# Patman86/SVT-AV1-Mod-by-Patman

Measured on AMD Instinct MI355X. Metric: encoded fps (4K 10-bit preset 8) + ME+txfm HBM GB/s vs roofline, 1/2/4/8 GPU, higher is better.
Workload: dtype u8 (ME) / int32 (transform)

## Files before the change

svt-av1-mod-by-patman_amd/csrc/me_frame.hip:

```cpp
#include <cstdio>
#include <cstdlib>
#include <cstring>

#include "common.hpp"
#include "sad_device.hpp"

using namespace svthip;
using namespace svthip::dev;

namespace {

#define NL 2
#define NR 4
#define MAX_SAD_VALUE_ (128 * 128 * 255)
#define MAX_U32_ 0xFFFFFFFFu

constexpr uint32_t ME_HME_WIN_DW = 3200;
constexpr uint32_t ME_WIN_DW     = ME_HME_WIN_DW - 64 * 16 - 256;
constexpr uint32_t fp_pitch_c(uint32_t tw) { return (((tw + 3) >> 2) + 17) | 1u; }
constexpr uint32_t FP_TILE_W = ME_WIN_DW / fp_pitch_c(64) >= 63 + 8 ? 64 : 32;
static_assert(ME_WIN_DW / fp_pitch_c(FP_TILE_W) >= 63 + 8, "full-pel window buffer too small for one tile");

struct PreHme {
    uint64_t sad;
    uint16_t sa_w, sa_h;
    int16_t  col, row;
    uint8_t  valid, pad_[7];
};

struct B64State {
    uint32_t org_x, org_y, b64_w, b64_h;
    SvtHipMeSearchResult sr[NL][NR];
    uint32_t reduce_div[NL][NR];
    uint32_t zz_sad[NL][NR];
    PreHme   ph[NL][NR][2];
    uint8_t  performed_phme[NL][NR][2];
    int16_t  l0x[NL][NR][2][2], l0y[NL][NR][2][2], l1x[NL][NR][2][2], l1y[NL][NR][2][2], l2x[NL][NR][2][2],
        l2y[NL][NR][2][2];
    uint64_t l0s[NL][NR][2][2], l1s[NL][NR][2][2], l2s[NL][NR][2][2];
    SvtHipSearchArea l0_min, l0_max;
    uint32_t wg_sum;
    int16_t  xc, yc, sw, sh, ox, oy;
    int32_t  do_centre, need_zero_sad, need_hme_sad;
    int16_t  stx, sty, stw, sth;
    int32_t  staged, restage;
    uint32_t zero_sad, hme_mv_sad;
    int16_t  fp_xc[NL * NR], fp_yc[NL * NR], fp_sw[NL * NR], fp_sh[NL * NR], fp_ox[NL * NR], fp_oy[NL * NR];
    uint8_t  fp_centre[NL * NR];
    uint32_t fp_inv[NL * NR];
    uint32_t first_ref_sad64;
    uint64_t me_sad_sum[NL][NR];
};

struct MeLds {
    static constexpr uint32_t WIN_DW = ME_WIN_DW, HME_WIN_DW = ME_HME_WIN_DW;
    SearchShared sh;
    B64State     st;
    union {
        alignas(16) uint32_t win[ME_HME_WIN_DW];
        struct {
            alignas(16) uint32_t fp_win_[ME_WIN_DW];
            alignas(16) uint32_t src_full[64 * 16];
            uint64_t bestkey[85];
            uint32_t me_dist[85];
        };
    };
    alignas(16) uint32_t src_q[32 * 8];
    alignas(16) uint32_t src_s[16 * 4];
};
static_assert(sizeof(MeLds::win) >= (ME_WIN_DW + 64 * 16) * 4 + 85 * 12, "full-pel view must fit the HME window buffer");

typedef __attribute__((address_space(1))) uint32_t g_u32;
#define MINV(a, b) ((a) < (b) ? (a) : (b))
#define MAXV(a, b) ((a) > (b) ? (a) : (b))
#define ABSV(a) ((a) < 0 ? -(a) : (a))

__device__ __forceinline__ uint32_t div_small(uint32_t x, uint32_t d) {
    return (d & (d - 1u)) == 0u && d ? x >> (31u - (uint32_t)__builtin_clz(d)) : x / d;
}

__device__ __forceinline__ uint16_t scaled_dist(uint16_t dist) {
    return (uint16_t)(((dist * 5) / 8) + ((dist % 8) == 0 ? 0 : 1));
}
__device__ __forceinline__ uint16_t pic_dist(const SvtHipMeParams &p, int li, int ri) {
    const int64_t d = (int64_t)p.picture_number - (int64_t)p.ref_picture_number[li][ri];
    return (uint16_t)(int16_t)ABSV(d);
}
__device__ __forceinline__ const uint8_t *plane_at(const SvtHipPlane8 &pl, int x, int y) {
    return pl.buf + (ptrdiff_t)((int)pl.org_y + y) * (ptrdiff_t)pl.stride + (int)pl.org_x + x;
}

__device__ __forceinline__ uint32_t block_sad16(const uint32_t *src, const uint8_t *ref, uint32_t ref_stride, uint32_t ndw, uint32_t rows,
                                                uint32_t row_step, uint32_t lane, uint32_t nlanes) {
    const uint32_t nch = (ndw + 3) >> 2, inv = make_inv_small(nch);
    uint32_t       acc = 0;
    for (uint32_t idx = lane; idx < nch * rows; idx += nlanes) {
        const uint32_t r = fast_div(idx, inv), ch = idx - r * nch;
        const uint4    sv = *(const uint4 *)&src[(r * row_step) * 16 + 4 * ch];
        const u128v    v  = load_u128_any(ref + (size_t)sad_mul_u24(r * row_step, ref_stride) + 16 * ch);
        const uint32_t nd = ndw - 4 * ch;
        acc = __builtin_amdgcn_sad_u8(sv.x, v.x, acc);
        acc = __builtin_amdgcn_sad_u8(sv.y, v.y, acc);
        if (nd > 2) {
            acc = __builtin_amdgcn_sad_u8(sv.z, v.z, acc);
            acc = __builtin_amdgcn_sad_u8(sv.w, v.w, acc);
        }
    }
    return acc;
}

template <class LDS>
__device__ void wg_block_sad(LDS &L, const uint8_t *ref, uint32_t ref_stride, uint32_t width, uint32_t rows,
                             uint32_t row_step) {
    if (threadIdx.x == 0)
        L.st.wg_sum = 0;
    __syncthreads();
    uint32_t acc = block_sad16(L.src_full, ref, ref_stride, width >> 2, rows, row_step, threadIdx.x, blockDim.x);
    acc = wave_sum(acc);
    if ((threadIdx.x & 63) == 0)
        atomicAdd(&L.st.wg_sum, acc);
    __syncthreads();
}

__device__ void hme_clamp(int16_t org_x, int16_t org_y, int16_t pad_w, int16_t pad_h, int16_t W, int16_t H, int16_t *pox,
                          int16_t *poy, int16_t *pw, int16_t *ph) {
    int16_t ox = *pox, oy = *poy, sa_w = *pw, sa_h = *ph;
    if ((org_x + ox) < -pad_w) {
        ox   = (int16_t)(-pad_w - org_x);
        sa_w = (int16_t)(sa_w - (-pad_w - (org_x + ox)));
    }
    if ((org_x + ox) > W - 1)
        ox = (int16_t)(ox - ((org_x + ox) - (W - 1)));
    if ((org_x + ox + sa_w) > W)
        sa_w = (int16_t)MAXV(1, sa_w - ((org_x + ox + sa_w) - W));
    sa_w = (sa_w < 8) ? sa_w : (int16_t)(sa_w & ~0x07);
    if ((org_y + oy) < -pad_h) {
        oy   = (int16_t)(-pad_h - org_y);
        sa_h = (int16_t)(sa_h - (-pad_h - (org_y + oy)));
    }
    if ((org_y + oy) > H - 1)
        oy = (int16_t)(oy - ((org_y + oy) - (H - 1)));
    if ((org_y + oy + sa_h) > H)
        sa_h = (int16_t)MAXV(1, sa_h - ((org_y + oy + sa_h) - H));
    *pox = ox, *poy = oy, *pw = sa_w, *ph = sa_h;
}

__device__ void set_desc(SearchDesc &d, const SvtHipMeParams &p, const SvtHipPlane8 &rp, int x_tl, int y_tl, int16_t sa_w,
                         int16_t sa_h, uint32_t skip) {
    const bool full = p.hme_search_method == 1;
    d.ref           = rp.buf + (ptrdiff_t)y_tl * (ptrdiff_t)rp.stride + x_tl;
    d.ref_stride    = full ? rp.stride : rp.stride * 2;
    d.raw_stride    = rp.stride;
    d.sa_w          = sa_w;
    d.sa_h          = sa_h;
    d.skip          = skip;
}

template <class SH>
__device__ void decode_result(const SH &sh, uint32_t i, bool sub, uint64_t *sad, int16_t *x, int16_t *y) {
    const uint64_t key = sh.best[i];
    uint64_t       s   = key >> 32;
    if (key != KEY_NONE) {
        const uint32_t idx = (uint32_t)key;
        *x = (int16_t)(idx & 0xffffu);
        *y = (int16_t)(idx >> 16);
    }
    if (sub)
        s *= 2;
    *sad = s;
}

__device__ void set_quadrants(int16_t x[2][2], int16_t y[2][2], uint64_t s[2][2], int16_t vx, int16_t vy, uint64_t vs) {
    for (int a = 0; a < 2; a++)
        for (int b = 0; b < 2; b++) x[a][b] = vx, y[a][b] = vy, s[a][b] = vs;
}

__device__ void best_quadrant(int16_t x[2][2], int16_t y[2][2], uint64_t s[2][2], int16_t *bx, int16_t *by, uint64_t *bs) {
    *bx = x[0][0], *by = y[0][0], *bs = s[0][0];
    if (s[1][0] < *bs) *bx = x[1][0], *by = y[1][0], *bs = s[1][0];
    if (s[0][1] < *bs) *bx = x[0][1], *by = y[0][1], *bs = s[0][1];
    if (s[1][1] < *bs) *bx = x[1][1], *by = y[1][1], *bs = s[1][1];
}

__device__ void clamp_me_window(int16_t xc, int16_t yc, int16_t ox_b, int16_t oy_b, int16_t W, int16_t H, int16_t pad, int16_t *psw,
                                int16_t *psh, int16_t *pox, int16_t *poy) {
    int16_t sw = *psw, sh_ = *psh;
    int16_t ox = (int16_t)(xc - (sw >> 1)), oy = (int16_t)(yc - (sh_ >> 1));
    ox  = ((ox_b + ox) < -pad) ? (int16_t)(-pad - ox_b) : ox;
    sw  = ((ox_b + ox) < -pad) ? (int16_t)(sw - (-pad - (ox_b + ox))) : sw;
    ox  = ((ox_b + ox) > W - 1) ? (int16_t)(ox - ((ox_b + ox) - (W - 1))) : ox;
    sw  = ((ox_b + ox + sw) > W) ? (int16_t)MAXV(1, sw - ((ox_b + ox + sw) - W)) : sw;
    sw  = (sw < 8) ? sw : (int16_t)(sw & ~0x07);
    oy  = ((oy_b + oy) < -pad) ? (int16_t)(-pad - oy_b) : oy;
    sh_ = ((oy_b + oy) < -pad) ? (int16_t)(sh_ - (-pad - (oy_b + oy))) : sh_;
    oy  = ((oy_b + oy) > H - 1) ? (int16_t)(oy - ((oy_b + oy) - (H - 1))) : oy;
    sh_ = ((oy_b + oy + sh_) > H) ? (int16_t)MAXV(1, sh_ - ((oy_b + oy + sh_) - H)) : sh_;
    *psw = sw, *psh = sh_, *pox = ox, *poy = oy;
}

__device__ __forceinline__ uint32_t fp_pitch(uint32_t tw) { return (((tw + 3) >> 2) + 17) | 1u; }

template <class LDS>
__device__ void fp_stage(LDS &L, const uint8_t *win_org, uint32_t stride, uint32_t tw, uint32_t th) {
    stage_rows16(L.win, fp_pitch(tw), win_org, stride, th + 63, blockDim.x, threadIdx.x);
    __syncthreads();
}

template <int CTRL> __device__ __forceinline__ uint32_t dpp_add(uint32_t v) {
    return v + (uint32_t)__builtin_amdgcn_update_dpp(0, (int)v, CTRL, 0xf, 0xf, false);
}

template <class LDS>
__device__ void fp_search(LDS &L, uint32_t pitch, uint32_t x0, uint32_t y0, uint32_t cw, uint32_t ch, uint32_t order0,
                          uint32_t order_pitch, bool sub) {
    const uint32_t tid = threadIdx.x;
    const uint32_t nq = (cw + 3) >> 2, nitems = nq * ch * 16, inv_nq = make_inv_small(nq);
    const uint32_t zo = tid & 15;
    const uint32_t zy = 2 * (zo >> 3) + ((zo >> 1) & 1), zx = 2 * ((zo >> 2) & 1) + (zo & 1);
    const uint32_t *s = &L.src_full[(16 * zy) * 16 + 4 * zx];
    for (uint32_t base = 0; base < nitems; base += blockDim.x) {
        if (base + (tid & ~63u) >= nitems)
            break;
        const uint32_t item = base + tid;
        const bool     on   = item < nitems;
        const uint32_t qi = on ? item >> 4 : 0, y = fast_div(qi, inv_nq), q = qi - sad_mul_u24(y, nq);
        const uint32_t *w = &L.win[sad_mul_u24(y0 + y + 16 * zy, pitch) + (x0 >> 2) + q + 4 * zx];
        uint64_t        a00 = 0, a01 = 0, a10 = 0, a11 = 0;
#pragma unroll
        for (uint32_t r = 0; r < 16; r++) {
            if (sub && (r & 1))
                continue;
            const uint32_t d0 = w[r * pitch], d1 = w[r * pitch + 1], d2 = w[r * pitch + 2], d3 = w[r * pitch + 3], d4 = w[r * pitch + 4];
            const uint4    sv = *(const uint4 *)&s[r * 16];
            if (r < 8) {
                a00 = __builtin_amdgcn_qsad_pk_u16_u8(pair64(d0, d1), sv.x, a00);
                a00 = __builtin_amdgcn_qsad_pk_u16_u8(pair64(d1, d2), sv.y, a00);
                a01 = __builtin_amdgcn_qsad_pk_u16_u8(pair64(d2, d3), sv.z, a01);
                a01 = __builtin_amdgcn_qsad_pk_u16_u8(pair64(d3, d4), sv.w, a01);
            } else {
                a10 = __builtin_amdgcn_qsad_pk_u16_u8(pair64(d0, d1), sv.x, a10);
                a10 = __builtin_amdgcn_qsad_pk_u16_u8(pair64(d1, d2), sv.y, a10);
                a11 = __builtin_amdgcn_qsad_pk_u16_u8(pair64(d2, d3), sv.z, a11);
                a11 = __builtin_amdgcn_qsad_pk_u16_u8(pair64(d3, d4), sv.w, a11);
            }
        }
        uint32_t k8[4] = {~0u, ~0u, ~0u, ~0u}, k16 = ~0u, k32 = ~0u, k64 = ~0u;
#pragma unroll
        for (uint32_t pp = 0; pp < 4; pp++) {
            const uint32_t lo_hi_shift = 16 * (pp & 1);
            const uint32_t c0 = ((pp < 2 ? (uint32_t)a00 : (uint32_t)(a00 >> 32)) >> lo_hi_shift) & 0xffff;
            const uint32_t c1 = ((pp < 2 ? (uint32_t)a01 : (uint32_t)(a01 >> 32)) >> lo_hi_shift) & 0xffff;
            const uint32_t c2 = ((pp < 2 ? (uint32_t)a10 : (uint32_t)(a10 >> 32)) >> lo_hi_shift) & 0xffff;
            const uint32_t c3 = ((pp < 2 ? (uint32_t)a11 : (uint32_t)(a11 >> 32)) >> lo_hi_shift) & 0xffff;
            const uint32_t s16 = c0 + c1 + c2 + c3;
            uint32_t       s32 = dpp_add<0xB1>(s16);
            s32                = dpp_add<0x4E>(s32);
            uint32_t s64       = dpp_add<0x124>(s32);
            s64                = dpp_add<0x128>(s64);
            if (4 * q + pp < cw) {
                k8[0] = min(k8[0], (c0 << 2) | pp), k8[1] = min(k8[1], (c1 << 2) | pp);
                k8[2] = min(k8[2], (c2 << 2) | pp), k8[3] = min(k8[3], (c3 << 2) | pp);
                k16 = min(k16, (s16 << 2) | pp), k32 = min(k32, (s32 << 2) | pp), k64 = min(k64, (s64 << 2) | pp);
            }
        }
        if (on && k16 != ~0u) {
            const uint32_t sh1 = sub ? 1 : 0;
            const uint32_t ord_row = order0 + sad_mul_u24(y, order_pitch) + 4 * q;
#define FP_KEY(k) (((unsigned long long)(((k) >> 2) << sh1) << 32) | (ord_row + ((k) & 3u)))
#pragma unroll
            for (uint32_t c = 0; c < 4; c++) atomicMin((unsigned long long *)&L.bestkey[21 + 4 * zo + c], FP_KEY(k8[c]));
            atomicMin((unsigned long long *)&L.bestkey[5 + zo], FP_KEY(k16));
            if ((zo & 3) == 0)
                atomicMin((unsigned long long *)&L.bestkey[1 + (zo >> 2)], FP_KEY(k32));
            if (zo == 0)
                atomicMin((unsigned long long *)&L.bestkey[0], FP_KEY(k64));
#undef FP_KEY
        }
    }
    __syncthreads();
}

__device__ const uint8_t z_to_raster_d[85] = {
    0,  1,  2,  3,  4,  5,  6,  9,  10, 7,  8,  11, 12, 13, 14, 17, 18, 15, 16, 19, 20, 21, 22, 29, 30, 23, 24, 31, 32,
    37, 38, 45, 46, 39, 40, 47, 48, 25, 26, 33, 34, 27, 28, 35, 36, 41, 42, 49, 50, 43, 44, 51, 52, 53, 54, 61, 62, 55,
    56, 63, 64, 69, 70, 77, 78, 71, 72, 79, 80, 57, 58, 65, 66, 59, 60, 67, 68, 73, 74, 81, 82, 75, 76, 83, 84};
__device__ __forceinline__ uint8_t pack_cand(uint32_t direction, uint32_t l0, uint32_t l1, uint32_t r0, uint32_t r1) {
    return (uint8_t)((direction & 3) | ((l0 & 3) << 2) | ((l1 & 3) << 4) | ((r0 & 1) << 6) | ((r1 & 1) << 7));
}
__device__ __forceinline__ int use_me_pu(const SvtHipMeParams &p, uint32_t n) {
    return p.enable_me_16x16 ? (p.enable_me_8x8 || n < 21) : (n < 5);
}

#define GS(li, ri, n) gs[((li) * NR + (ri)) * 85 + (n)]
#define GM(li, ri, n) gm[((li) * NR + (ri)) * 85 + (n)]

template <class LDS>
// ... 820 lines not shown
        fp_stage(L, plane_at(rp, ox_b + S.stx, oy_b + S.sty), rp.stride, (uint32_t)S.stw, (uint32_t)S.sth);
        fp_search(L, fp_pitch((uint32_t)S.stw), (uint32_t)(S.xc - S.stx), (uint32_t)(S.yc - S.sty), 1, 1, 0, 1, me_sub);
        if (tid < 64) {
            const uint32_t v    = (uint32_t)(L.bestkey[21 + tid] >> 32);
            const uint32_t mean = (uint32_t)(L.bestkey[0] >> 32) / 64;
            const int32_t  dv   = (int32_t)v - (int32_t)mean;
            const uint32_t ssq  = wave_sum((uint32_t)(dv * dv));
            if (tid == 0) {
                int16_t        sw = S.sw, sh_ = S.sh;
                const uint32_t var = ssq / 64;
                if (var > p.me_sr_mult2_th) {
                    sw  = (int16_t)((MAXV(1, sw * 3 / 2) + 7) & ~0x7);
                    sh_ = (int16_t)MAXV(1, sh_ * 3 / 2);
                }
                if (var < p.me_sr_div4_th) {
                    sw  = (int16_t)((MAXV(1, sw >> 2) + 7) & ~0x7);
                    sh_ = (int16_t)MAXV(1, sh_ >> 2);
                    sh_ = (int16_t)MAXV(3, sh_);
                } else if (var < p.me_sr_div2_th) {
                    sw  = (int16_t)((MINV(sw, sw >> 1) + 7) & ~0x7);
                    sh_ = (int16_t)MINV(sh_, sh_ >> 1);
                    sh_ = (int16_t)MAXV(3, sh_);
                }
                S.sw = sw, S.sh = sh_;
            }
        }
        __syncthreads();
    }
    if (tid == 0) {
        int16_t sw = S.sw, sh_ = S.sh, ox, oy;
        clamp_me_window(S.xc, S.yc, ox_b, oy_b, W, H, pad, &sw, &sh_, &ox, &oy);
        S.sw = sw, S.sh = sh_, S.ox = ox, S.oy = oy;
        S.restage = !(S.staged && ox >= S.stx && oy >= S.sty && ox + (sw > 0 ? sw : 0) <= S.stx + S.stw &&
                      oy + (sh_ > 0 ? sh_ : 0) <= S.sty + S.sth && ((ox - S.stx) & 3) == 0);
    }
    __syncthreads();
    }
    {
        const int      ox = S.ox, oy = S.oy;
        const uint32_t sw = (uint32_t)(S.sw > 0 ? S.sw : 0), sh_ = (uint32_t)(S.sh > 0 ? S.sh : 0);
        if (!S.restage) {
            fp_search(L, fp_pitch((uint32_t)S.stw), (uint32_t)(ox - S.stx), (uint32_t)(oy - S.sty), sw, sh_, 1, sw, me_sub);
        } else {
            const uint32_t tw = sw < FP_TILE_W ? sw : FP_TILE_W;
            const uint32_t pitch_t = fp_pitch(tw);
            uint32_t       th      = tw ? MINV(sh_, LDS::WIN_DW / pitch_t - 63) : 0;
            for (uint32_t ty = 0; th && ty < sh_; ty += th)
                for (uint32_t tx = 0; tx < sw; tx += tw) {
                    const uint32_t cw = MINV(tw, sw - tx), ch = MINV(th, sh_ - ty);
                    fp_stage(L, plane_at(rp, ox_b + ox + (int)tx, oy_b + oy + (int)ty), rp.stride, cw, ch);
                    fp_search(L, fp_pitch(cw), 0, 0, cw, ch, 1 + ty * sw + tx, sw, me_sub);
                }
        }
        uint32_t part = 0;
        for (uint32_t pu = tid; pu < 85; pu += blockDim.x) {
            const uint64_t key    = L.bestkey[pu];
            const uint32_t ord    = (uint32_t)key;
            const uint32_t my_sad = (uint32_t)(key >> 32);
            if (li == 0 && ri == 0 && pu == 0)
                S.first_ref_sad64 = my_sad;
            if (pu >= 21)
                part += my_sad;
            if (!store)
                continue;
            gs[(li * NR + ri) * 85 + pu] = my_sad;
            if (ord != 0xffffffffu) {
                int16_t mx, my;
                if (ord == 0) {
                    mx = S.xc, my = S.yc;
                } else {
                    const uint32_t pos = ord - 1, row = prepared ? fast_div(pos, S.fp_inv[li * NR + ri]) : pos / sw;
                    mx = (int16_t)((int)(pos - row * sw) + ox), my = (int16_t)((int)row + oy);
                }
                gm[(li * NR + ri) * 85 + pu] = ((uint32_t)(uint16_t)my << 16) | (uint16_t)mx;
            }
        }
        part = wave_sum(part);
        if (store && (tid & 63) == 0 && part)
            atomicAdd((unsigned long long *)&S.me_sad_sum[li][ri], (unsigned long long)part);
    }
    __syncthreads();
}

template <class LDS>
__device__ void me_prune_lane0(LDS &L, const Ctx &c) {
    ME_CTX_LOCALS(c);
    if (tid < 64) {
        const Slot            q   = slot_of(tid, p, nlists);
        SvtHipMeSearchResult &r   = S.sr[q.li][q.ri];
        uint64_t              sad = q.slot ? r.hme_sad : ~(uint64_t)0;
        if (q.searched) {
            sad       = r.do_ref ? S.me_sad_sum[q.li][q.ri] : (uint64_t)(MAX_SAD_VALUE_ * 64);
            r.hme_sad = sad;
        }
        const uint16_t th = p.prune_ref_if_me_sad_dev_bigger_than_th;
        if (th != (uint16_t)~0) {
            const uint64_t best = slots_min(sad);
            if (q.slot && q.ri >= 1 && (sad - best) * 100 > (th * best))
                r.do_ref = 0;
        }
    }
}

template <class LDS>
__device__ void finalize_b64(LDS &L, const Ctx &c) {
    ME_CTX_LOCALS(c);
    const uint32_t b64 = c.b64;
    const SvtHipMeFrameOut &out    = job.out;
    const uint32_t          stored = p.enable_me_16x16 ? (p.enable_me_8x8 ? 85u : 21u) : 5u;
    uint32_t               *o_mv   = out.me_mv_array + (size_t)b64 * stored * p.max_refs;
    uint8_t                *o_cand = out.me_candidate_array + (size_t)b64 * stored * p.max_cand;
    uint8_t                *o_tot  = out.total_me_candidate_index + (size_t)b64 * stored;
    const bool single = p.num_of_ref_pic_to_search[0] == 1 && p.num_of_ref_pic_to_search[1] == 0;
    const bool mrpoff = p.num_of_ref_pic_to_search[0] == 1 && p.num_of_ref_pic_to_search[1] == 1;
    if ((single || mrpoff) && tid < stored)
        o_tot[tid] = 1;
    __syncthreads();
    if (tid < p.max_number_of_pus_per_sb && tid < 85) {
        if (single)
            cand_single_ref(L, p, gs, gm, tid, o_mv, o_cand);
        else if (mrpoff)
            cand_mrp_off(L, p, gs, gm, tid, (uint32_t)nlists, o_mv, o_cand, o_tot);
        else
            cand_general(L, p, gs, gm, tid, (uint32_t)nlists, o_mv, o_cand, o_tot);
    }
    __syncthreads();

    if (tid < 64) {
        const uint32_t e8 = L.me_dist[21 + tid];
        const uint32_t d8 = wave_sum_all(e8);
        const uint32_t d16 = wave_sum_all(tid < 16 ? L.me_dist[5 + tid] : 0u), d32 = wave_sum_all(tid < 4 ? L.me_dist[1 + tid] : 0u);
        const uint64_t mean = d8 / 64;
        const int64_t  dv   = (int64_t)e8 - (int64_t)mean;
        const uint64_t sq   = (uint64_t)(dv * dv);
        const uint32_t lo = wave_sum_all((uint32_t)sq & 0xffffu), mid = wave_sum_all((uint32_t)(sq >> 16) & 0xffffu),
                       hi = wave_sum_all((uint32_t)(sq >> 32) & 0xffffu), top = wave_sum_all((uint32_t)(sq >> 48));
        if (tid == 0) {
            const uint64_t ssq = (uint64_t)lo + ((uint64_t)mid << 16) + ((uint64_t)hi << 32) + ((uint64_t)top << 48);
            const uint32_t d64 = L.me_dist[0];
            const uint32_t pix = b64_w * b64_h;
            out.me_8x8_cost_variance[b64] = (uint32_t)(ssq / 64);
            out.rc_me_distortion[b64]     = p.input_resolution_le_480p ? d8 : d16;
            out.me_64x64_distortion[b64]  = div_small(d64 * 4096u, pix);
            out.me_32x32_distortion[b64]  = div_small(d32 * 4096u, pix);
            out.me_16x16_distortion[b64]  = div_small(d16 * 4096u, pix);
            out.me_8x8_distortion[b64]    = div_small(d8 * 4096u, pix);
        }
    }
    if (tid < NL * NR)
        out.search_results[(size_t)b64 * NL * NR + tid] = (&S.sr[0][0])[tid];
}


#ifdef SVT_HIP_ME_ABLATE
__device__ int g_me_stop = 99;
#define ME_STOP(k)          \
    do {                    \
        if (me_stop == (k)) \
            return;         \
    } while (0)
#else
#define ME_STOP(k) \
    do {           \
    } while (0)
#endif

// ... 14 lines not shown
    if (!make_ctx(c, sjob, blockIdx.x))
        return;
#ifdef SVT_HIP_ME_ABLATE
    const int me_stop = g_me_stop;
#endif
    ME_CTX_LOCALS(c);
    stage_sources(L, c, 7);
    for (uint32_t i = tid; i < NL * NR * 85; i += blockDim.x) gs[i] = 0, gm[i] = 0;
    init_state_lane0(L, c);
    __syncthreads();
    ME_PHASE(0);
    ME_STOP(0);
    if (p.me_early_exit_th || p.me_safe_limit_zz_th) {
        zz_sad_all(L, c);
        zz_prune_lane0(L, c);
        __syncthreads();
    }
    ME_PHASE(1);
    ME_STOP(1);
    {
        const bool pre = p.prehme_enable, split = nlists == 2 && (p.prehme_l1_early_exit || tl == 0);
        const bool l0 = p.enable_hme_flag && p.enable_hme_level0_flag, l1 = p.enable_hme_flag && p.enable_hme_level1_flag;
        const bool l2 = p.enable_hme_flag && p.enable_hme_level2_flag;
        const bool dep = p.enable_me_sr_adjustment && p.distance_based_hme_resizing && p.reduce_hme_l0_sr_th_min &&
            p.reduce_hme_l0_sr_th_max && nref > 1;
        for (int step = 0; step < 6; step++) {
            if (step == 2) {
                if (pre) {
                    phme_prune_lane0(L, c);
                    __syncthreads();
                }
                ME_PHASE(2);
                ME_STOP(2);
            } else if (step == 4) {
                ME_PHASE(3);
                ME_STOP(3);
            } else if (step == 5) {
                ME_PHASE(4);
                ME_STOP(4);
                if (pre || l0 || l1) {
                    stage_sources(L, c, 1);
                    __syncthreads();
                }
            }
            const bool active = step == 0 ? pre : step == 1 ? (pre && split) : step == 2 ? l0 : step == 3 ? (l0 && dep) : step == 4 ? l1 : l2;
            if (!active)
                continue;
            const int f0 = step == 1 ? R0 : (step == 3 ? 1 : 0);
            const int f1 = step == 0 ? (split ? R0 : nref) : (step == 2 ? (dep ? 1 : nref) : nref);
            SearchArgs a;
            for (int part = 0; part < 2; part++) {
                if (step < 2)
                    prehme_round(L, c, f0, f1, step == 0 || tl > 0, part, a);
                else if (step < 4)
                    hme_l0_round(L, c, f0, f1, part, a);
                else if (step == 4)
                    hme_l1_round(L, c, f0, f1, part, a);
                else
                    hme_l2_round(L, c, f0, f1, part, a);
                if (part == 0 && a.search) {
                    ME_SITE(step < 2 ? 0 : (step < 4 ? 1 : step - 2));
#if SVT_HIP_ME_L1_DIRECT
                    const int direct_rows = step == 4 ? wg_direct_plan(L.sh, a.nd, a.src, a.row_dw, a.bw, a.bh) : -1;
                    if (direct_rows >= 0)
                        wg_direct_search(L.sh, a.nd, (uint32_t)direct_rows, a.src, a.row_dw, a.bh);
                    else
#endif
                    wg_multi_search(L.sh, a.nd, a.src, a.row_dw, a.bw, a.bh, L.win, a.cap);
                }
            }
        }
    }
    ME_PHASE(5);
    ME_STOP(5);
    centre_prune_lane0(L, c);
    __syncthreads();
    ME_PHASE(6);
    ME_STOP(6);
    const bool tf_exit = p.me_mctf && S.sr[0][0].hme_sad < p.tf_me_exit_th;
    if (!tf_exit) {
        const bool prepared = p.me_early_exit_th != 0;
        if (prepared)
            fullpel_prepare_all(L, c);
        for (int li = 0; li < nlists; ++li)
            for (int ri = 0; ri < p.num_of_ref_pic_to_search[li]; ++ri)
                if (S.sr[li][ri].do_ref)
                    fullpel_ref(L, c, li, ri, true, prepared);
    }
    ME_PHASE(7);
    ME_STOP(7);
    if (p.me_mctf) {
        if (tid < NL * NR)
            job.out.search_results[(size_t)c.b64 * NL * NR + tid] = (&S.sr[0][0])[tid];
        return;
    }
    if (p.enable_hme_flag && p.enable_me_hme_ref_pruning) {
        me_prune_lane0(L, c);
        __syncthreads();
    }
    ME_PHASE(8);
    finalize_b64(L, c);
    ME_PHASE(10);
}

}

#ifdef SVT_HIP_ME_ABLATE
extern "C" __attribute__((visibility("default"))) int32_t svt_hip_debug_me_stop(int32_t k) {
    SVT_HIP_CHECK(hipDeviceSynchronize());
    const int32_t stop = k & 0xff, skip = k >> 8;
    SVT_HIP_CHECK(hipMemcpyToSymbol(HIP_SYMBOL(g_me_stop), &stop, sizeof(stop)));
    SVT_HIP_CHECK(hipMemcpyToSymbol(HIP_SYMBOL(g_ms_skip), &skip, sizeof(skip)));
    return SVT_HIP_OK;
}
#endif

#ifdef SVT_HIP_ME_PROFILE
extern "C" __attribute__((visibility("default"))) int32_t svt_hip_debug_me_profile(unsigned long long out[32], int32_t reset) {
    SVT_HIP_CHECK(hipDeviceSynchronize());
    SVT_HIP_CHECK(hipMemcpyFromSymbol(out, HIP_SYMBOL(g_me_prof), sizeof(unsigned long long) * 11));
    SVT_HIP_CHECK(hipMemcpyFromSymbol(out + 16, HIP_SYMBOL(g_ms_prof), sizeof(unsigned long long) * 16));
    if (reset) {
        unsigned long long z[16] = {};
        SVT_HIP_CHECK(hipMemcpyToSymbol(HIP_SYMBOL(g_me_prof), z, sizeof(z)));
        SVT_HIP_CHECK(hipMemcpyToSymbol(HIP_SYMBOL(g_ms_prof), z, sizeof(unsigned long long) * 16));
    }
    return SVT_HIP_OK;
}
#endif

extern "C" uint32_t svt_hip_me_b64_count(uint32_t width, uint32_t height) {
    const uint32_t aw = (width + 7u) & ~7u, ah = (height + 7u) & ~7u;
    return ((aw + 63) / 64) * ((ah + 63) / 64);
}

static int32_t validate_job(const SvtHipMeFrameJob &j, uint32_t idx) {
    const SvtHipMeParams &p = j.prm;
    auto bad = [&](const char *what) { return refuse("svt_hip_me_frames: job %u: %s", idx, what); };
    if (p.num_hme_sa_w != 2 || p.num_hme_sa_h != 2)
        return bad("num_hme_sa_w/h must be 2 (as in the reference, motion_estimation.c:1945)");
    if (p.num_of_list_to_search < 1 || p.num_of_list_to_search > 2)
        return bad("num_of_list_to_search must be 1 or 2");
    for (int l = 0; l < 2; l++)
        if (p.num_of_ref_pic_to_search[l] > SVT_HIP_ME_MAX_REF)
            return bad("too many reference pictures");
    if (p.num_of_ref_pic_to_search[0] < 1)
        return bad("list 0 needs at least one reference");
    if (p.max_number_of_pus_per_sb != 85)
        return bad("max_number_of_pus_per_sb must be 85 (SQUARE_PU_COUNT)");
    if (p.max_refs == 0 || p.max_cand == 0)
        return bad("max_refs / max_cand not set");
    if (!j.src.full.buf || !j.src.quarter.buf || !j.src.sixteenth.buf)
        return bad("source pyramid incomplete");
    if (j.src.full.width < 64 || j.src.full.height < 64 || j.src.full.width > 16384 || j.src.full.height > 8704)
        return bad("unsupported picture size");
    if (j.src.full.org_x < 64 || j.src.full.org_y < 64)
        return bad("full-resolution planes need >= 64 samples of padding");
    auto pyramid_ok = [](const SvtHipPyramid8 &y) {
        const SvtHipPlane8 *pl[3] = {&y.full, &y.quarter, &y.sixteenth};
        const uint32_t      pad[3] = {64, 32, 16};
        for (int i = 0; i < 3; i++) {
            if (pl[i]->org_x < pad[i] || pl[i]->org_y < pad[i])
                return false;
            if (pl[i]->width != (y.full.width >> i) || pl[i]->height != (y.full.height >> i))
                return false;
            if (pl[i]->stride < (uint32_t)pl[i]->width + 2u * pl[i]->org_x)
                return false;
        }
        return true;
    };
// ... 98 lines not shown
```

svt-av1-mod-by-patman_amd/csrc/sad_device.hpp:

```cpp
#pragma once

#include <hip/hip_runtime.h>
#include <stdint.h>

namespace svthip {
namespace dev {

constexpr int      WG_THREADS = 256;
constexpr int      MAX_SEARCH = 32;
constexpr uint32_t SEG_ALIGN  = 4;
constexpr uint64_t KEY_NONE   = ((uint64_t)0xffffffu << 32) | 0xffffffffu;
constexpr int      MAX_PASS   = 9;

struct SearchDesc {
    const uint8_t *ref;
    uint32_t       ref_stride;
    uint32_t       raw_stride;
    int32_t        sa_w, sa_h;
    uint32_t       skip;
    uint32_t k;
    uint32_t fast;
    uint32_t nq;
    uint32_t no;
    uint32_t n_srows;
    uint32_t pitch_dw;
    uint32_t rows_per_pos;
    uint32_t inv_no;
    int16_t  aux_x, aux_y;
    uint32_t aux_go;
};

struct SearchSeg {
    uint32_t d;
    uint32_t j0, nj;
    uint32_t lds_dw;
    uint32_t nstage;
    uint32_t item_base;
};

template <int NS> struct SearchSharedT {
    static constexpr int MAXS = NS;
    SearchDesc desc[NS];
    SearchSeg  seg[NS];
    uint64_t   best[NS];
    uint32_t   nseg, nitems, nstage_dw;
    uint32_t   next_d, next_j;
    uint32_t   npass;
    uint32_t   pass_item0[MAX_PASS + 1];
    uint8_t    pass_seg0[MAX_PASS + 3];
#ifdef SVT_HIP_ME_PROFILE
    uint32_t   prof_site;
#endif
};
using SearchShared = SearchSharedT<MAX_SEARCH>;

#ifdef SVT_HIP_ME_ABLATE
static __device__ int g_ms_skip;
#endif
#ifdef SVT_HIP_ME_PROFILE
static __device__ unsigned long long g_ms_prof[16];
#define MS_PHASE(i)                                                 \
    do {                                                            \
        if (threadIdx.x == 0) {                                     \
            const unsigned long long t_ = wall_clock64();           \
            atomicAdd(&g_ms_prof[(sh.prof_site & 3u) * 4 + i], t_ - ms_last);                 \
            ms_last = t_;                                           \
        }                                                           \
    } while (0)
#else
#define MS_PHASE(i) \
    do {            \
    } while (0)
#endif

__device__ __forceinline__ uint64_t pair64(uint32_t lo, uint32_t hi) { return ((uint64_t)hi << 32) | lo; }
typedef uint32_t __attribute__((aligned(1))) u32_unaligned;
__device__ __forceinline__ uint32_t load_u32_any(const uint8_t *g) {
    return *(const __attribute__((address_space(1))) u32_unaligned *)g;
}
typedef uint32_t __attribute__((ext_vector_type(4), aligned(1))) u128_unaligned;
typedef uint32_t __attribute__((ext_vector_type(4))) u128v;
__device__ __forceinline__ u128v load_u128_any(const uint8_t *g) {
    return *(const __attribute__((address_space(1))) u128_unaligned *)g;
}

extern "C" __device__ unsigned sad_mul_u24(unsigned, unsigned) __asm("llvm.amdgcn.mul.u24");

__device__ __forceinline__ void stage_rows16(uint32_t *__restrict__ w0, uint32_t pitch, const uint8_t *g0, uint32_t rstride,
                                             uint32_t rows, uint32_t lanes, uint32_t lid) {
    const uint32_t nch = (pitch + 3) >> 2;
    const uint32_t lg  = nch <= 2 ? 1u : (nch <= 4 ? 2u : (nch <= 8 ? 3u : (nch <= 16 ? 4u : 5u)));
    const uint32_t lpr = 1u << lg, rpi = lanes >> lg;
    const uint32_t c0 = lid & (lpr - 1), r0 = lid >> lg;
    for (uint32_t ch = c0; ch < nch; ch += lpr) {
        const uint32_t  nd = pitch - 4 * ch;
        const uint8_t  *g  = g0 + 16 * ch;
        uint32_t       *w  = w0 + 4 * ch;
        for (uint32_t row = r0; row < rows; row += 2 * rpi) {
            const uint32_t row1 = row + rpi;
            const bool     two  = row1 < rows;
            const u128v    a    = load_u128_any(g + (size_t)sad_mul_u24(row, rstride));
            u128v          b    = {0u, 0u, 0u, 0u};
            if (two)
                b = load_u128_any(g + (size_t)sad_mul_u24(row1, rstride));
            uint32_t *wa = w + sad_mul_u24(row, pitch), *wb = w + sad_mul_u24(row1, pitch);
            wa[0] = a.x;
            if (nd > 1) wa[1] = a.y;
            if (nd > 2) wa[2] = a.z;
            if (nd > 3) wa[3] = a.w;
            if (two) {
                wb[0] = b.x;
                if (nd > 1) wb[1] = b.y;
                if (nd > 2) wb[2] = b.z;
                if (nd > 3) wb[3] = b.w;
            }
        }
    }
}

__device__ __forceinline__ uint32_t fast_div(uint32_t n, uint32_t inv) { return inv ? __umulhi(n, inv) : n; }
__device__ __forceinline__ uint32_t make_inv(uint32_t d) { return d > 1 ? 0xffffffffu / d + 1u : 0u; }
__device__ const uint32_t INV_SMALL[65] = {
    0u, 0u, 0x80000000u, 0x55555556u, 0x40000000u, 0x33333334u, 0x2aaaaaabu, 0x24924925u, 0x20000000u, 0x1c71c71du, 0x1999999au, 0x1745d175u, 0x15555556u,
    0x13b13b14u, 0x12492493u, 0x11111112u, 0x10000000u, 0x0f0f0f10u, 0x0e38e38fu, 0x0d79435fu, 0x0ccccccdu, 0x0c30c30du, 0x0ba2e8bbu, 0x0b21642du, 0x0aaaaaabu,
    0x0a3d70a4u, 0x09d89d8au, 0x097b425fu, 0x0924924au, 0x08d3dcb1u, 0x08888889u, 0x08421085u, 0x08000000u, 0x07c1f07du, 0x07878788u, 0x07507508u, 0x071c71c8u,
    0x06eb3e46u, 0x06bca1b0u, 0x06906907u, 0x06666667u, 0x063e7064u, 0x06186187u, 0x05f417d1u, 0x05d1745eu, 0x05b05b06u, 0x0590b217u, 0x0572620bu, 0x05555556u,
    0x0539782au, 0x051eb852u, 0x05050506u, 0x04ec4ec5u, 0x04d4873fu, 0x04bda130u, 0x04a7904bu, 0x04924925u, 0x047dc120u, 0x0469ee59u, 0x0456c798u, 0x04444445u,
    0x04325c54u, 0x04210843u, 0x04104105u, 0x04000000u};
__device__ __forceinline__ uint32_t make_inv_small(uint32_t d) { return d <= 64 ? INV_SMALL[d] : make_inv(d); }

__device__ __forceinline__ void quad_sad(const uint32_t *__restrict__ w, uint32_t w_row_dw,
                                         const uint32_t *__restrict__ s, uint32_t s_row_dw, uint32_t bw, uint32_t bh,
                                         uint32_t out[4]) {
    const uint32_t nfull = bw >> 2, tail = bw & 3;
    const uint32_t rows_per_flush = nfull ? (64u / nfull ? 64u / nfull : 1u) : 64u;
    const uint32_t tmask          = tail ? ((1u << (8 * tail)) - 1u) : 0u;
    uint32_t       a0 = 0, a1 = 0, a2 = 0, a3 = 0;
    uint64_t       acc = 0;
    uint32_t       since = 0;
    for (uint32_t r = 0; r < bh; r++) {
        const uint32_t *wr = w + r * w_row_dw;
        const uint32_t *sr = s + r * s_row_dw;
        uint32_t        lo = wr[0];
        for (uint32_t i = 0; i < nfull; i++) {
            const uint32_t hi = wr[i + 1];
#ifdef SVT_HIP_NO_QSAD
            a0 = __builtin_amdgcn_sad_u8(lo, sr[i], a0);
            a1 = __builtin_amdgcn_sad_u8(__builtin_amdgcn_alignbyte(hi, lo, 1u), sr[i], a1);
            a2 = __builtin_amdgcn_sad_u8(__builtin_amdgcn_alignbyte(hi, lo, 2u), sr[i], a2);
            a3 = __builtin_amdgcn_sad_u8(__builtin_amdgcn_alignbyte(hi, lo, 3u), sr[i], a3);
#else
            acc = __builtin_amdgcn_qsad_pk_u16_u8(pair64(lo, hi), sr[i], acc);
#endif
            lo = hi;
        }
        if (tail) {
            const uint32_t hi = wr[nfull + 1];
            const uint32_t sv = sr[nfull] & tmask;
            a0 = __builtin_amdgcn_sad_u8(lo & tmask, sv, a0);
            a1 = __builtin_amdgcn_sad_u8(__builtin_amdgcn_alignbyte(hi, lo, 1u) & tmask, sv, a1);
            a2 = __builtin_amdgcn_sad_u8(__builtin_amdgcn_alignbyte(hi, lo, 2u) & tmask, sv, a2);
            a3 = __builtin_amdgcn_sad_u8(__builtin_amdgcn_alignbyte(hi, lo, 3u) & tmask, sv, a3);
        }
        if (++since == rows_per_flush) {
            a0 += (uint32_t)(acc & 0xffff), a1 += (uint32_t)((acc >> 16) & 0xffff);
            a2 += (uint32_t)((acc >> 32) & 0xffff), a3 += (uint32_t)(acc >> 48);
// ... 517 lines not shown
```

Before: 6086.

## Add direct-from-global full-pel search across all refs for small windows

Adds a full-pel ME path that, when every searched reference has a small window (at most 24 wide by 9 rows), skips staging each reference window into LDS. It instead reads reference pixels straight from global memory with unaligned vector loads and qsad instructions, spreading work groups across all references in one pass. Per-partition best keys are merged with LDS atomicMin. The aim is to remove the per-reference LDS staging and barriers, at the cost of more global/L2 reads and atomics. The path is on by default but only taken when early-exit preparation is enabled and the windows fit; otherwise the old per-reference loop runs.

Result: faster. 6327, median of 6 (+4.0%).

```diff
diff --git a/svt-av1-mod-by-patman_amd/csrc/me_frame.hip b/svt-av1-mod-by-patman_amd/csrc/me_frame.hip
--- a/svt-av1-mod-by-patman_amd/csrc/me_frame.hip
+++ b/svt-av1-mod-by-patman_amd/csrc/me_frame.hip
@@ -20,6 +20,12 @@
 constexpr uint32_t fp_pitch_c(uint32_t tw) { return (((tw + 3) >> 2) + 17) | 1u; }
 constexpr uint32_t FP_TILE_W = ME_WIN_DW / fp_pitch_c(64) >= 63 + 8 ? 64 : 32;
 static_assert(ME_WIN_DW / fp_pitch_c(FP_TILE_W) >= 63 + 8, "full-pel window buffer too small for one tile");
+
+#ifndef SVT_HIP_ME_FP_DIRECT
+#define SVT_HIP_ME_FP_DIRECT 1
+#endif
+constexpr uint32_t FPD_MAX_W = 24, FPD_MAX_ROWS = 9, FPD_MAX_GROUPS = NL * NR * ((FPD_MAX_W + 7) / 8) * FPD_MAX_ROWS;
+static_assert(FPD_MAX_GROUPS <= 256, "one thread per group of work items sets the direct search up");
 
 struct PreHme {
     uint64_t sad;
@@ -59,7 +65,13 @@
     union {
         alignas(16) uint32_t win[ME_HME_WIN_DW];
         struct {
-            alignas(16) uint32_t fp_win_[ME_WIN_DW];
+            union {
+                alignas(16) uint32_t fp_win_[ME_WIN_DW];
+                struct {
+                    uint64_t fpd_key[NL * NR][85];
+                    uint2    fpd_grp[FPD_MAX_GROUPS];
+                };
+            };
             alignas(16) uint32_t src_full[64 * 16];
             uint64_t bestkey[85];
             uint32_t me_dist[85];
@@ -69,6 +81,8 @@
     alignas(16) uint32_t src_s[16 * 4];
 };
 static_assert(sizeof(MeLds::win) >= (ME_WIN_DW + 64 * 16) * 4 + 85 * 12, "full-pel view must fit the HME window buffer");
+static_assert(sizeof(MeLds::fpd_key) + sizeof(MeLds::fpd_grp) <= sizeof(MeLds::fp_win_), "direct full-pel view must fit the window buffer");
+static_assert(SVT_HIP_ME_MAX_REF == NR && SVT_HIP_ME_MAX_LIST == NL, "reference slot = list * NR + index");
 
 typedef __attribute__((address_space(1))) uint32_t g_u32;
 #define MINV(a, b) ((a) < (b) ? (a) : (b))
@@ -211,7 +225,7 @@
 }
 
 template <class LDS>
-__device__ void fp_search(LDS &L, uint32_t pitch, uint32_t x0, uint32_t y0, uint32_t cw, uint32_t ch, uint32_t order0,
+__device__ __forceinline__ void fp_search(LDS &L, uint32_t pitch, uint32_t x0, uint32_t y0, uint32_t cw, uint32_t ch, uint32_t order0,
                           uint32_t order_pitch, bool sub) {
     const uint32_t tid = threadIdx.x;
     const uint32_t nq = (cw + 3) >> 2, nitems = nq * ch * 16, inv_nq = make_inv_small(nq);
@@ -1198,6 +1212,172 @@
     __syncthreads();
 }
 
+#if SVT_HIP_ME_FP_DIRECT
+
+__device__ __forceinline__ void fpd_rows(const uint8_t *gp, uint32_t gstep, const uint32_t *__restrict__ s, uint32_t sstep, uint32_t nrows,
+                                         uint64_t a[4]) {
+#pragma unroll 1
+    for (uint32_t r = 0; r < nrows; r++) {
+        const u128v v  = load_u128_any(gp);
+        const u64v  w  = load_u64_any(gp + 16);
+        const uint4 sv = *(const uint4 *)s;
+        a[0] = __builtin_amdgcn_qsad_pk_u16_u8(pair64(v.x, v.y), sv.x, a[0]);
+        a[0] = __builtin_amdgcn_qsad_pk_u16_u8(pair64(v.y, v.z), sv.y, a[0]);
+        a[1] = __builtin_amdgcn_qsad_pk_u16_u8(pair64(v.z, v.w), sv.z, a[1]);
+        a[1] = __builtin_amdgcn_qsad_pk_u16_u8(pair64(v.w, w.x), sv.w, a[1]);
+        a[2] = __builtin_amdgcn_qsad_pk_u16_u8(pair64(v.y, v.z), sv.x, a[2]);
+        a[2] = __builtin_amdgcn_qsad_pk_u16_u8(pair64(v.z, v.w), sv.y, a[2]);
+        a[3] = __builtin_amdgcn_qsad_pk_u16_u8(pair64(v.w, w.x), sv.z, a[3]);
+        a[3] = __builtin_amdgcn_qsad_pk_u16_u8(pair64(w.x, w.y), sv.w, a[3]);
+        gp += gstep, s += sstep;
+    }
+}
+
+template <class LDS>
+__device__ __forceinline__ bool fullpel_direct_all(LDS &L, const Ctx &c) {
+    ME_CTX_LOCALS(c);
+    const uint32_t lane = tid & 63u, wv = tid >> 6;
+    uint32_t ng = 0;
+    {
+        const Slot q   = slot_of(lane, p, nlists);
+        bool       bad = false;
+        if (q.searched && S.sr[q.li][q.ri].do_ref) {
+            const int sw = S.fp_sw[lane], sh_ = S.fp_sh[lane];
+            bad = sw > (int)FPD_MAX_W || sh_ > (int)FPD_MAX_ROWS;
+            if (sw > 0 && sh_ > 0)
+                ng = (((uint32_t)sw + 7) >> 3) * (uint32_t)sh_;
+        }
+        if (__ballot(bad))
+            return false;
+    }
+    uint32_t incl = ng;
+    incl += (uint32_t)__builtin_amdgcn_update_dpp(0, (int)incl, 0x111, 0xf, 0xf, true);
+    incl += (uint32_t)__builtin_amdgcn_update_dpp(0, (int)incl, 0x112, 0xf, 0xf, true);
+    incl += (uint32_t)__builtin_amdgcn_update_dpp(0, (int)incl, 0x114, 0xf, 0xf, true);
+    const uint32_t ngroups = (uint32_t)__builtin_amdgcn_readlane((int)incl, NL * NR - 1);
+    uint32_t end[NL * NR - 1];
+#pragma unroll
+    for (int k = 0; k < NL * NR - 1; k++) end[k] = (uint32_t)__builtin_amdgcn_readlane((int)incl, k);
+    if (tid < ngroups) {
+        uint32_t g = 0, base = 0;
+#pragma unroll
+        for (int k = 0; k < NL * NR - 1; k++)
+            if (tid >= end[k])
+                g = (uint32_t)k + 1, base = end[k];
+        const SvtHipPlane8 &rp  = job.ref[g / NR][g % NR].full;
+        const uint32_t      gsw = (uint32_t)S.fp_sw[g], no = (gsw + 7) >> 3, loc = tid - base;
+        const uint32_t      y = fast_div(loc, make_inv_small(no)), o = loc - y * no;
+        const int           px = (int)rp.org_x + (int)(int16_t)org_x + S.fp_ox[g] + (int)(8 * o);
+        const int           py = (int)rp.org_y + (int)(int16_t)org_y + S.fp_oy[g] + (int)y;
+        const uint32_t      nv = gsw - 8 * o < 8 ? gsw - 8 * o : 8;
+        L.fpd_grp[tid]         = make_uint2((uint32_t)(py * (int)rp.stride + px), g | (nv << 3) | ((1 + y * gsw + 8 * o) << 8));
+    }
+    for (uint32_t g = wv; g < (uint32_t)(NL * NR); g += blockDim.x >> 6) {
+        const uint32_t li = g / NR, ri = g % NR;
+        if (!((int)li < nlists && ri < p.num_of_ref_pic_to_search[li] && S.sr[li][ri].do_ref))
+            continue;
+        uint64_t *const key = L.fpd_key[g];
+        if (S.fp_centre[g]) {
+            const uint32_t sh1 = me_sub ? 1u : 0u;
+            const uint32_t v   = ((const uint16_t *)L.src_q)[g * 64 + lane];
+            uint32_t       s16 = dpp_add<0xB1>(v);
+            s16                = dpp_add<0x4E>(s16);
+            uint32_t s32       = dpp_add<0x124>(s16);
+            s32                = dpp_add<0x128>(s32);
+            const uint32_t s64 = wave_sum_all(v);
+            key[21 + lane] = (uint64_t)(v << sh1) << 32;
+            if ((lane & 3) == 0)
+                key[5 + (lane >> 2)] = (uint64_t)(s16 << sh1) << 32;
+            if ((lane & 15) == 0)
+                key[1 + (lane >> 4)] = (uint64_t)(s32 << sh1) << 32;
+            if (lane == 0)
+                key[0] = (uint64_t)(s64 << sh1) << 32;
+        } else {
+            for (uint32_t pu = lane; pu < 85; pu += 64) key[pu] = ((uint64_t)MAX_SAD_VALUE_ << 32) | 0xffffffffu;
+        }
+    }
+    __syncthreads();
+    {
+        const uint32_t zo = tid & 15;
+        const uint32_t zy = 2 * (zo >> 3) + ((zo >> 1) & 1), zx = 2 * ((zo >> 2) & 1) + (zo & 1);
+        const uint32_t *s = &L.src_full[(16 * zy) * 16 + 4 * zx];
+        const uint32_t sh1 = me_sub ? 1u : 0u;
+        for (uint32_t item = tid; item < 16 * ngroups; item += blockDim.x) {
+            const uint2         rec = L.fpd_grp[item >> 4];
+            const uint32_t      g = rec.y & 7u, nv = (rec.y >> 3) & 15u, ord_row = rec.y >> 8;
+            const SvtHipPlane8 &rp = job.ref[g / NR][g % NR].full;
+            const uint32_t      stride = rp.stride;
+            const uint8_t      *w = rp.buf + rec.x + sad_mul_u24(16 * zy, stride) + 16 * zx;
+            uint64_t            at[4] = {0, 0, 0, 0}, ab[4] = {0, 0, 0, 0};
+            fpd_rows(w, stride << sh1, s, 16u << sh1, 8u >> sh1, at);
+            fpd_rows(w + 8 * stride, stride << sh1, s + 8 * 16, 16u << sh1, 8u >> sh1, ab);
+            uint32_t k8[4] = {~0u, ~0u, ~0u, ~0u}, k16 = ~0u, k32 = ~0u, k64 = ~0u;
+#pragma unroll
+            for (uint32_t pp = 0; pp < 8; pp++) {
+                const uint32_t qd = 2 * (pp >> 2), lo_hi_shift = 16 * (pp & 1);
+                const uint32_t c0 = (((pp & 2) ? (uint32_t)(at[qd] >> 32) : (uint32_t)at[qd]) >> lo_hi_shift) & 0xffff;
+                const uint32_t c1 = (((pp & 2) ? (uint32_t)(at[qd + 1] >> 32) : (uint32_t)at[qd + 1]) >> lo_hi_shift) & 0xffff;
+                const uint32_t c2 = (((pp & 2) ? (uint32_t)(ab[qd] >> 32) : (uint32_t)ab[qd]) >> lo_hi_shift) & 0xffff;
+                const uint32_t c3 = (((pp & 2) ? (uint32_t)(ab[qd + 1] >> 32) : (uint32_t)ab[qd + 1]) >> lo_hi_shift) & 0xffff;
+                const uint32_t s16 = c0 + c1 + c2 + c3;
+                uint32_t       s32 = dpp_add<0xB1>(s16);
+                s32                = dpp_add<0x4E>(s32);
+                uint32_t s64       = dpp_add<0x124>(s32);
+                s64                = dpp_add<0x128>(s64);
+                const uint32_t tag = pp < nv ? pp : (0xff800000u | pp);
+                k8[0] = min(k8[0], (c0 << 3) | tag), k8[1] = min(k8[1], (c1 << 3) | tag);
+                k8[2] = min(k8[2], (c2 << 3) | tag), k8[3] = min(k8[3], (c3 << 3) | tag);
+                k16 = min(k16, (s16 << 3) | tag), k32 = min(k32, (s32 << 3) | tag), k64 = min(k64, (s64 << 3) | tag);
+            }
+            uint64_t *const key = L.fpd_key[g];
+#define FP_KEY(k) (((unsigned long long)(((k) >> 3) << sh1) << 32) | (ord_row + ((k) & 7u)))
+#pragma unroll
+            for (uint32_t cq = 0; cq < 4; cq++) atomicMin((unsigned long long *)&key[21 + 4 * zo + cq], FP_KEY(k8[cq]));
+            atomicMin((unsigned long long *)&key[5 + zo], FP_KEY(k16));
+            if ((zo & 3) == 0)
+                atomicMin((unsigned long long *)&key[1 + (zo >> 2)], FP_KEY(k32));
+            if (zo == 0)
+                atomicMin((unsigned long long *)&key[0], FP_KEY(k64));
+#undef FP_KEY
+        }
+    }
+    __syncthreads();
+    for (uint32_t g = wv; g < (uint32_t)(NL * NR); g += blockDim.x >> 6) {
+        const uint32_t li = g / NR, ri = g % NR;
+        if (!((int)li < nlists && ri < p.num_of_ref_pic_to_search[li] && S.sr[li][ri].do_ref))
+            continue;
+        const int      ox = S.fp_ox[g], oy = S.fp_oy[g];
+        const uint32_t sw = (uint32_t)(S.fp_sw[g] > 0 ? S.fp_sw[g] : 0);
+        uint32_t       part = 0;
+        for (uint32_t pu = lane; pu < 85; pu += 64) {
+            const uint64_t key    = L.fpd_key[g][pu];
+            const uint32_t ord    = (uint32_t)key;
+            const uint32_t my_sad = (uint32_t)(key >> 32);
+            if (g == 0 && pu == 0)
+                S.first_ref_sad64 = my_sad;
+            if (pu >= 21)
+                part += my_sad;
+            gs[g * 85 + pu] = my_sad;
+            if (ord != 0xffffffffu) {
+                int16_t mx, my;
+                if (ord == 0) {
+                    mx = S.fp_xc[g], my = S.fp_yc[g];
+                } else {
+                    const uint32_t pos = ord - 1, row = fast_div(pos, S.fp_inv[g]);
+                    mx = (int16_t)((int)(pos - row * sw) + ox), my = (int16_t)((int)row + oy);
+                }
+                gm[g * 85 + pu] = ((uint32_t)(uint16_t)my << 16) | (uint16_t)mx;
+            }
+        }
+        part = wave_sum(part);
+        if (lane == 0 && part)
+            S.me_sad_sum[li][ri] += (uint64_t)part;
+    }
+    __syncthreads();
+    return true;
+}
+#endif
+
 template <class LDS>
 __device__ void me_prune_lane0(LDS &L, const Ctx &c) {
     ME_CTX_LOCALS(c);
@@ -1378,10 +1558,16 @@
         const bool prepared = p.me_early_exit_th != 0;
         if (prepared)
             fullpel_prepare_all(L, c);
-        for (int li = 0; li < nlists; ++li)
-            for (int ri = 0; ri < p.num_of_ref_pic_to_search[li]; ++ri)
-                if (S.sr[li][ri].do_ref)
-                    fullpel_ref(L, c, li, ri, true, prepared);
+        bool direct = false;
+#if SVT_HIP_ME_FP_DIRECT
+        if (prepared)
+            direct = fullpel_direct_all(L, c);
+#endif
+        if (!direct)
+            for (int li = 0; li < nlists; ++li)
+                for (int ri = 0; ri < p.num_of_ref_pic_to_search[li]; ++ri)
+                    if (S.sr[li][ri].do_ref)
+                        fullpel_ref(L, c, li, ri, true, prepared);
     }
     ME_PHASE(7);
     ME_STOP(7);
diff --git a/svt-av1-mod-by-patman_amd/csrc/sad_device.hpp b/svt-av1-mod-by-patman_amd/csrc/sad_device.hpp
--- a/svt-av1-mod-by-patman_amd/csrc/sad_device.hpp
+++ b/svt-av1-mod-by-patman_amd/csrc/sad_device.hpp
@@ -82,6 +82,11 @@
 typedef uint32_t __attribute__((ext_vector_type(4))) u128v;
 __device__ __forceinline__ u128v load_u128_any(const uint8_t *g) {
     return *(const __attribute__((address_space(1))) u128_unaligned *)g;
+}
+typedef uint32_t __attribute__((ext_vector_type(2), aligned(1))) u64_unaligned;
+typedef uint32_t __attribute__((ext_vector_type(2))) u64v;
+__device__ __forceinline__ u64v load_u64_any(const uint8_t *g) {
+    return *(const __attribute__((address_space(1))) u64_unaligned *)g;
 }
 
 extern "C" __device__ unsigned sad_mul_u24(unsigned, unsigned) __asm("llvm.amdgcn.mul.u24");
```
